# rajashree-srikanth/drone-sim-python

Hardware: AMD Instinct MI355X
Metric: trajectory-optimisations/sec (6-seg poly, 50 wpts) (higher is better)
Workload: dtype f64 residual/gradient + f32 MFMA J^T J

## Files before the change

### drone-sim-python_amd/csrc/fit_device.h

```cpp
#pragma once
#include <hip/hip_runtime.h>

#include "../../include/d2d.h"

#define FIT_G 9.81
#define FIT_OBS_K 2.0
#define FIT_OBS_ARGMAX 3.4538776394910684

typedef float f32x4 __attribute__((ext_vector_type(4)));
typedef float f32x2 __attribute__((ext_vector_type(2)));

__device__ __forceinline__ void wave_lds_sync() {
  __builtin_amdgcn_fence(__ATOMIC_RELEASE, "wavefront");
  __builtin_amdgcn_wave_barrier();
  __builtin_amdgcn_fence(__ATOMIC_ACQUIRE, "wavefront");
}

__device__ __forceinline__ double uniform_d(double v) {
  const int lo = __builtin_amdgcn_readfirstlane(__double2loint(v));
  const int hi = __builtin_amdgcn_readfirstlane(__double2hiint(v));
  return __hiloint2double(hi, lo);
}
__device__ __forceinline__ int uniform_i(int v) { return __builtin_amdgcn_readfirstlane(v); }

// ... 170 lines not shown
}

__device__ __forceinline__ ScenP load_scenp(const double *__restrict__ p) {
  ScenP s;
  s.cv = p[PR_CV]; s.cphi = p[PR_CPHI]; s.cobs = p[PR_COBS]; s.k0 = p[PR_K0]; s.k1 = p[PR_K1];
  s.cv2 = p[PR_CV2]; s.cphi2 = p[PR_CPHI2]; s.wb2 = p[PR_WB2]; s.wwp = p[PR_WWP]; s.wbnd = p[PR_WBND];
  s.vsp = p[PR_VSP]; s.wx = p[PR_WX]; s.wy = p[PR_WY]; s.phimax = p[PR_PHIMAX]; s.vmin = p[PR_VMIN]; s.vmax = p[PR_VMAX];
  s.o0x = p[PR_O0X]; s.o0y = p[PR_O0Y]; s.o1x = p[PR_O1X]; s.o1y = p[PR_O1Y];
  s.ccol = p[PR_CCOL]; s.kc = p[PR_KC]; s.pmask = (int)p[PR_PMASK];
  s.c0 = p[PR_C0]; s.c1 = p[PR_C1]; s.cphimax = p[PR_CPHIMAX];
  s.ext = p + PR_EXT;
  return s;
}

#define FIT_PK 8
__device__ __forceinline__ void prepk_entry(const double *__restrict__ pr, const double *__restrict__ Gp64, int K, int k,
                                            double o[FIT_PK]) {
#pragma unroll
  for (int d = 0; d < 3; ++d) {
    const double *gp = Gp64 + ((size_t)d * K + k) * 4;
    double ax = 0.0, ay = 0.0;
#pragma unroll
    for (int c = 0; c < 4; ++c) { ax = fma(gp[c], pr[PR_DX + c], ax); ay = fma(gp[c], pr[PR_DY + c], ay); }
    o[2 * d] = ax; o[2 * d + 1] = ay;
  }
  const int n1 = K / 2, n2 = K - n1;
  if (k < n1) {
    o[6] = (k == n1 - 1 && n1 > 1) ? pr[PR_P2X] : k * pr[PR_SAX] + pr[PR_X0];
    o[7] = (k == n1 - 1 && n1 > 1) ? pr[PR_P2Y] : k * pr[PR_SAY] + pr[PR_Y0];
  } else {
    const int i = k - n1;
    o[6] = (i == n2 - 1 && n2 > 1) ? pr[PR_X1] : i * pr[PR_SBX] + pr[PR_P2X];
    o[7] = (i == n2 - 1 && n2 > 1) ? pr[PR_Y1] : i * pr[PR_SBY] + pr[PR_P2Y];
  }
}

__device__ __forceinline__ int q_slot(int lane, int nq) { return lane < nq ? 2 * lane : 2 * (lane - nq) + 1; }

template <int NQ>
__device__ __forceinline__ void flat_outputs_pk(const FitGeom &g, const double *__restrict__ G64,
                                                const double *__restrict__ q, const double pk[FIT_PK], int k, double Y[6]) {
  typedef double __attribute__((ext_vector_type(2), may_alias)) f64x2a;
  const int nq = NQ ? NQ : g.nq, gstr = NQ ? NQ + 1 : g.gstr;
#pragma unroll
  for (int c = 0; c < 6; ++c) Y[c] = pk[c];
  const double *g0 = G64 + (size_t)k * gstr;
  const double *g1 = g0 + (size_t)g.K * gstr;
  const double *g2 = g1 + (size_t)g.K * gstr;
  int j = 0;
// ... 263 lines not shown
```

### drone-sim-python_amd/csrc/fit_kernels.hip

```cpp
#include <algorithm>
#include <chrono>
#include <cmath>
#include <cstdlib>
#include <cstring>
#include <vector>

#include "fit_device.h"
#include "fit_phases.h"
#include "fit_seg.h"
#include "fit_plan.h"
#include "fit_handout_prior.h"

#define FIT_EVAL_WPB_MAX 16
#define FIT_WPB_MAX 12
#define FIT_THREADS (64 * FIT_WPB_MAX)
#define FIT_LDS_BYTES (160 * 1024)
#define FIT_LDS_STATIC 256


struct FitLds {
  int G64, G32, wave0, wave_stride;
  int q, u, coef, cfd;
  int total;
};
// ... 23 lines not shown
}

static bool pick_eval_layout(int K, int nq, bool *g32_lds, int *wpb, int nds = 0) {
  for (int pass = 0; pass < 2; ++pass) {
    const bool in_lds = pass == 0;
    for (int w = FIT_EVAL_WPB_MAX; w >= (in_lds ? 4 : 1); --w)
      if (eval_lds_layout(K, nq, in_lds, w, nds).total <= FIT_LDS_BYTES - FIT_LDS_STATIC) { *g32_lds = in_lds; *wpb = w; return true; }
  }
  return false;
}

__device__ __forceinline__ void stage(void *dst, const void *src, int bytes) {
  double *d = reinterpret_cast<double *>(dst);
  const double *s = reinterpret_cast<const double *>(src);
  for (int i = threadIdx.x; i < bytes / 8; i += blockDim.x) d[i] = s[i];
}

__global__ void __launch_bounds__(256)
fit_prep_kernel(int B, int K, double duration, const double *__restrict__ scen, double *__restrict__ prep) {
  const int b = blockIdx.x * blockDim.x + threadIdx.x;
  if (b >= B) return;
  prep_row(scen + (size_t)b * D2D_SCEN_STRIDE, duration, K, prep + (size_t)b * FIT_PREP_STRIDE);
}

__global__ void __launch_bounds__(256)
fit_prepk_kernel(int B, int K, const double *__restrict__ prep, const double *__restrict__ Gp64, double *__restrict__ pk) {
  const long i = blockIdx.x * (long)blockDim.x + threadIdx.x;
  if (i >= (long)B * K) return;
  const int b = i / K, k = i - (long)b * K;
  double o[FIT_PK];
  prepk_entry(prep + (size_t)b * FIT_PREP_STRIDE, Gp64, K, k, o);
#pragma unroll
  for (int c = 0; c < FIT_PK; ++c) pk[((size_t)b * FIT_PK + c) * K + k] = o[c];
}

template <int NB, int NQ, bool G32_LDS>
__global__ void __launch_bounds__(64 * FIT_EVAL_WPB_MAX)
// ... 1434 lines not shown
#pragma unroll
      for (int t = 0; t < NT; ++t) acc[t] = f32x4{0.f, 0.f, 0.f, 0.f};
#pragma unroll
      for (int s = 0; s < D2D_FIT_MAX_S; ++s)
        if (s < sa.m.S) segment_project<NB, NQ>(nq, Zl32, s, bs[s][0], lane, acc);
      float *Hb = H_out + (size_t)b * NT * 256;
#pragma unroll
      for (int t = 0; t < NT; ++t)
#pragma unroll
        for (int r = 0; r < 4; ++r) Hb[(t * 4 + r) * 64 + lane] = acc[t][r];
    }
    wave_lds_sync();
  }
}

__global__ void __launch_bounds__(256)
fit_state_init_kernel(int B, int off, int stride, double *__restrict__ lm, int32_t *__restrict__ flags,
                      int32_t *__restrict__ queue) {
  const int i = blockIdx.x * blockDim.x + threadIdx.x;
  if (i == 0 && queue) { queue[0] = 0; queue[1] = 0; queue[2] = 0; queue[3] = 0; queue[4] = 0; queue[5] = 0; }
  if (i >= B) return;
  const int b = off + i * stride;
  lm[LM_STRIDE * b + 0] = D2D_LM_LAMBDA0; lm[LM_STRIDE * b + 1] = 2.0; lm[LM_STRIDE * b + 2] = 0.0; lm[LM_STRIDE * b + 3] = 0.0;
  lm[LM_STRIDE * b + 4] = 0.0; lm[LM_STRIDE * b + 5] = -1.0; lm[LM_STRIDE * b + 6] = 2.0; lm[LM_STRIDE * b + 7] = 0.0;
  flags[4 * b + FL_STATUS] = D2D_ST_RUNNING; flags[4 * b + FL_ITERS] = 0; flags[4 * b + FL_NEED] = 1;
  if (stride == 1) flags[4 * b + FL_NEVAL] = 0;
}


#define ORDER_BINS 2048
__global__ void __launch_bounds__(1024)
fit_order_kernel(int B, const int32_t *__restrict__ iters, int32_t *__restrict__ order) {
  __shared__ int hist[ORDER_BINS];
  for (int i = threadIdx.x; i < ORDER_BINS; i += blockDim.x) hist[i] = 0;
  __syncthreads();
  for (int b = threadIdx.x; b < B; b += blockDim.x) {
    int k = iters[b];
    k = k < 0 ? 0 : (k >= ORDER_BINS ? ORDER_BINS - 1 : k);
    atomicAdd(&hist[ORDER_BINS - 1 - k], 1);
  }
  __syncthreads();
// ... 9 lines not shown
      part[cur ^ 1][t] = v;
      cur ^= 1;
      __syncthreads();
    }
    const int excl = part[cur][t] - (h0 + h1);
    hist[2 * t] = excl; hist[2 * t + 1] = excl + h0;
  }
  __syncthreads();
  for (int b = threadIdx.x; b < B; b += blockDim.x) {
    int k = iters[b];
    k = k < 0 ? 0 : (k >= ORDER_BINS ? ORDER_BINS - 1 : k);
    order[atomicAdd(&hist[ORDER_BINS - 1 - k], 1)] = b;
  }
}

__global__ void __launch_bounds__(256)
fit_handout_key_kernel(int B, double duration, const double *__restrict__ scen, const float *__restrict__ tab, int32_t *__restrict__ key) {
  const int b = blockIdx.x * blockDim.x + threadIdx.x;
  if (b >= B) return;
  const double *r = scen + (size_t)b * D2D_SCEN_STRIDE;
  const double dx = r[D2D_SC_X1] - r[D2D_SC_X0], dy = r[D2D_SC_Y1] - r[D2D_SC_Y0];
  const double d = sqrt(dx * dx + dy * dy), D = r[D2D_SC_VREF] * duration;
  const double h = 0.5 * sqrt(fmax(D * D - d * d, 0.0));
  const double gl = r[D2D_SC_GOLEFT] > 0.0 ? 1.0 : (r[D2D_SC_GOLEFT] < 0.0 ? -1.0 : 0.0);
  const double beta = atan2(dy, dx), a = atan2(gl * h, 0.5 * d);
  const double TWO_PI = 6.283185307179586, PI = 3.141592653589793;
  auto wrap = [&](double v) { v = fmod(v + PI, TWO_PI); if (v < 0.0) v += TWO_PI; return v; };
  auto abin = [&](double v) { int i = (int)(wrap(v) * (D2D_HANDOUT_NB / TWO_PI)); return i < 0 ? 0 : (i >= D2D_HANDOUT_NB ? D2D_HANDOUT_NB - 1 : i); };
  const int b0 = abin(r[D2D_SC_PSI0] - (beta + a)), b1 = abin(r[D2D_SC_PSI1] - (beta - a));
  const double x = D > 0.0 ? d / D : 0.0;
  int bx = (int)floor((x - D2D_HANDOUT_X_LO) * (D2D_HANDOUT_ND / (D2D_HANDOUT_X_HI - D2D_HANDOUT_X_LO)));
  bx = bx < 0 ? 0 : (bx >= D2D_HANDOUT_ND ? D2D_HANDOUT_ND - 1 : bx);
  float k = tab[b0 * D2D_HANDOUT_ND + bx] + tab[(D2D_HANDOUT_NB + b1) * D2D_HANDOUT_ND + bx];
  if (!(k == k)) k = 0.f;
  int ki = (int)(8.f * (k + 40.f));
  key[b] = ki < 0 ? 0 : (ki >= ORDER_BINS ? ORDER_BINS - 1 : ki);
}

__global__ void __launch_bounds__(256)
fit_pos_kernel(int B, FitGeom g, const double *__restrict__ G64, const double *__restrict__ Gp64,
               const double *__restrict__ prep, const double *__restrict__ q, double *__restrict__ pos) {
  const long i = blockIdx.x * (long)blockDim.x + threadIdx.x;
  if (i >= (long)B * g.K) return;
  const int b = i / g.K, k = i - (long)b * g.K;
  const double *pr = prep + (size_t)b * FIT_PREP_STRIDE;
  const double *qa = q + (size_t)b * 2 * g.nq;
  const double *gp = Gp64 + (size_t)k * 4, *g0 = G64 + (size_t)k * g.gstr;
  double x = 0.0, y = 0.0;
  for (int c = 0; c < 4; ++c) { x = fma(gp[c], pr[PR_DX + c], x); y = fma(gp[c], pr[PR_DY + c], y); }
  for (int j = 0; j < g.nq; ++j) { x = fma(g0[j], qa[j], x); y = fma(g0[j], qa[g.nq + j], y); }
  pos[((size_t)b * 2) * g.K + k] = x;
// ... 40 lines not shown
    const int st = flags[4 * b + FL_STATUS];
    nr = (st == D2D_ST_CONVERGED || st == D2D_ST_STALLED) ? 0.0 : 1.0;
    ne = 0.5 * flags[4 * b + FL_NEVAL];
  }
  c = wave_sum(c); gm = wave_max(gm); nr = wave_sum(nr); ne = wave_sum(ne);
  if ((threadIdx.x & 63) == 0) {
    atomicAdd(&stats[0], c);
    atomicAdd(&stats[2], nr);
    atomicAdd(&stats[3], ne);
    atomicMax(reinterpret_cast<unsigned long long *>(&stats[1]), (unsigned long long)__double_as_longlong(gm));
  }
}

__global__ void __launch_bounds__(256)
fit_export_kernel(int B, const int32_t *__restrict__ flags, int32_t *__restrict__ iters,
                  int32_t *__restrict__ status) {
  const int b = blockIdx.x * blockDim.x + threadIdx.x;
  if (b >= B) return;
  if (iters) iters[b] = flags[4 * b + FL_ITERS];
  if (status) status[b] = flags[4 * b + FL_STATUS];
}

__global__ void __launch_bounds__(256)
fit_init_kernel(int B, int K, int nq, double duration, const double *__restrict__ Gp,
                const double *__restrict__ Pinit, const double *__restrict__ scen,
                double *__restrict__ q) {
  const int wave = threadIdx.x >> 6, lane = threadIdx.x & 63;
  const int b = blockIdx.x * 4 + wave;
  if (b >= B) return;
  const Scen s = load_scen(scen + (size_t)b * D2D_SCEN_STRIDE, duration);
  const int n = 2 * nq;
  for (int l = lane; l < n; l += 64) {
    const int ax = l >= nq, j = l - ax * nq;
// ... 120 lines not shown
  {
    int cap = 64;
    while (cap < B) cap <<= 1;
    SCRATCH_ALLOC(d_ring, (size_t)cap * sizeof(int32_t))
    pl->ring_cap = cap;
  }
  SCRATCH_ALLOC(d_cost, (size_t)B * sizeof(double))
  SCRATCH_ALLOC(d_lm, (size_t)B * LM_STRIDE * sizeof(double))
  SCRATCH_ALLOC(d_flags, (size_t)B * 4 * sizeof(int32_t))
#undef SCRATCH_ALLOC
  if (int rc = fit_knot_ensure(pl, B)) { free_scratch(pl); return rc; }
  pl->cap_B = B;
  return D2D_OK;
}

static int launch_prep(d2d_ctx *ctx, const d2d_fit_plan *pl, int B, const double *scen) {
  const_cast<d2d_fit_plan *>(pl)->rows_B = 0;
  hipLaunchKernelGGL(fit_prep_kernel, dim3((B + 63) / 64), dim3(64), 0, ctx->stream, B, pl->K, pl->duration, scen, pl->d_prep);
  hipLaunchKernelGGL(fit_prepk_kernel, dim3(((long)B * pl->K + 255) / 256), dim3(256), 0, ctx->stream, B, pl->K, pl->d_prep, pl->d_Gp, pl->d_pk);
  D2D_LAUNCH_CHECK();
  return D2D_OK;
}

static GroupArgs no_groups() { return GroupArgs{nullptr, 0, 0, 1, 0}; }

static int launch_eval(d2d_ctx *ctx, const d2d_fit_plan *pl, int B, const double *q,
                       int32_t *flags, double *cost, double *g, float *H, GroupArgs ga = no_groups(),
                       f32x4 *rows = nullptr) {
  const FitGeom gm = geom_of(pl);
  const FitLds L = eval_lds_layout(pl->K, pl->nq, pl->g32_lds, pl->wpb_eval, pl->nds);
  const int NB = (2 * pl->nq + 15) / 16;
  int nblk = (B + pl->wpb_eval - 1) / pl->wpb_eval;
  if (nblk > pl->n_cu) nblk = pl->n_cu;
  const dim3 grid(nblk), block(64 * pl->wpb_eval);
  static const int dbg = getenv("D2D_FIT_ABLATE") ? atoi(getenv("D2D_FIT_ABLATE")) : 0;
#define LAUNCH_EVAL(NBV, INLDS)                                                                    \
// ... 35 lines not shown
}

static int lm_slice(const d2d_fit_opts &o) { return o.slice > 0 ? o.slice : 0; }

static int solve_kernel_of(const d2d_fit_plan *pl, const d2d_fit_opts &o) {
  if (!pl->use_lm) return 2;
  return (pl->kn.wpb > 0 && o.mode == D2D_LM_MODE_MINPACK && lm_slice(o) <= 0) ? 1 : 0;
}

static const int32_t *handout_order(const d2d_fit_plan *pl, int B) {
  if (pl->order_B == B) return pl->d_order;
  if (pl->last_order == pl->d_order_pred && pl->last_order_B == B) return pl->d_order_pred;
  return nullptr;
}

static int launch_handout(d2d_ctx *ctx, d2d_fit_plan *pl, int B, const double *scen) {
  hipLaunchKernelGGL(fit_handout_key_kernel, dim3((B + 255) / 256), dim3(256), 0, ctx->stream, B, pl->duration, scen, pl->d_hprior, pl->d_hkey);
  hipLaunchKernelGGL(fit_order_kernel, dim3(1), dim3(1024), 0, ctx->stream, B, pl->d_hkey, pl->d_order_pred);
  D2D_LAUNCH_CHECK();
  return D2D_OK;
}

static int launch_lm(d2d_ctx *ctx, const d2d_fit_plan *pl, int B, double *q, const d2d_fit_opts &o, int iter_cap) {
  const FitGeom gm = geom_of(pl);
  const FusedLds L = fused_lds_layout(pl->K, pl->nq, 48, pl->wpb_lm);
  static const bool want_stamps = getenv("D2D_LM_STAMPS") != nullptr;
  static const bool want_times = getenv("D2D_LM_TIMES") != nullptr;
  std::chrono::steady_clock::time_point t0;
  if (want_times) { D2D_CHECK_HIP(hipStreamSynchronize(ctx->stream)); t0 = std::chrono::steady_clock::now(); }
  unsigned long long *stamps = want_stamps ? reinterpret_cast<unsigned long long *>(ctx->stats_dev + 8) : nullptr;
  if (want_stamps) D2D_CHECK_HIP(hipMemsetAsync(stamps, 0, 13 * sizeof(unsigned long long), ctx->stream));
  const int blocks = B < pl->n_cu ? B : pl->n_cu;
// ... 440 lines not shown
    out[2 * pl->prof_kind[i]] += ms;
    out[2 * pl->prof_kind[i] + 1] += 1.0;
  }
  return D2D_OK;
}


int d2d_fit_begin(d2d_ctx *ctx, d2d_fit_plan *pl, int B) {
  D2D_REQUIRE(ctx && pl, "d2d_fit_begin: null argument");
  D2D_REQUIRE(B >= 1, "d2d_fit_begin: B must be >= 1");
  if (pl->active_B != 0 && B > pl->cap_B) {
    d2d_set_error("d2d_fit_begin: a begin/iterate sequence of %d trajectories is in progress on this plan (finish it first)", pl->active_B);
    return D2D_ESTATE;
  }
  if (int rc = ensure_scratch(pl, B)) return rc;
  hipLaunchKernelGGL(fit_state_init_kernel, dim3((B + 255) / 256), dim3(256), 0, ctx->stream, B, 0, 1, pl->d_lm, pl->d_flags, ctx->counter_dev + 8);
  D2D_LAUNCH_CHECK();
  D2D_CHECK_HIP(hipMemsetAsync(pl->d_ring, 0xff, (size_t)pl->ring_cap * sizeof(int32_t), ctx->stream));
  pl->it_done = 0;
  pl->active_B = B;
  pl->solve_q = nullptr; pl->solve_kernel = -1;
  pl->last_order = nullptr; pl->last_order_B = 0;
  pl->prep_valid_for = nullptr;
  pl->rows_B = 0;
  pl->last_slice = 0; pl->last_running = -1;
  pl->gsweeps_R = 0;
  return D2D_OK;
}

int d2d_fit_iterate(d2d_ctx *ctx, d2d_fit_plan *pl, int B, const double *scen, double *q,
                    const d2d_fit_opts *opts, int n_iters, int32_t *n_running) {
  D2D_REQUIRE(ctx && pl && scen && q, "d2d_fit_iterate: null argument");
  if (pl->active_B != B) { d2d_set_error("d2d_fit_iterate: call d2d_fit_begin(B=%d) first", B); return D2D_ESTATE; }
  const d2d_fit_opts o = opts_or_default(opts);
  D2D_REQUIRE(o.max_iter >= 1 && n_iters >= 1, "d2d_fit_iterate: max_iter and n_iters must be >= 1");
  const dim3 g1((B + 255) / 256), b1(256);
  if (pl->prep_valid_for != scen) {
    if (int rc = launch_prep(ctx, pl, B, scen)) return rc;
    pl->prep_valid_for = scen;
  }
  if ((pl->use_lm || pl->use_long) && pl->n_group <= 1) {
    const int sk = solve_kernel_of(pl, o);
    if (pl->solve_kernel < 0) {
      pl->solve_q = q; pl->solve_kernel = sk;
      pl->last_order = pl->order_B == B ? pl->d_order : nullptr;
      if (pl->order_B != B && pl->has_prior && o.handout == D2D_HANDOUT_PREDICTED && o.mode == D2D_LM_MODE_MINPACK && B > 8 * pl->n_cu) {
        if (int rc = launch_handout(ctx, pl, B, scen)) return rc;
        pl->last_order = pl->d_order_pred;
      }
      pl->last_order_B = pl->last_order ? B : 0;
    } else {
      if (q != pl->solve_q) {
        d2d_set_error("d2d_fit_iterate: q differs from the buffer this solve started on (between d2d_fit_begin and d2d_fit_finish the solve owns q)");
        return D2D_EINVAL;
      }
      if (sk != pl->solve_kernel) {
        d2d_set_error("d2d_fit_iterate: these options (mode / slice) would move the solve in progress to another kernel; finish it and begin again");
        return D2D_ESTATE;
      }
    }
    int budget = o.max_iter - pl->it_done;
    if (budget > n_iters) budget = n_iters;
// ... 49 lines not shown
      return D2D_ESTATE;
    }
    if (int rc = launch_lm(ctx, pl, B, q, pl->last_opts, cap)) return rc;
  }
}

int d2d_fit_finish(d2d_ctx *ctx, d2d_fit_plan *pl, int B, const double *scen, const double *q,
                   double *cost, int32_t *iters, int32_t *status, double *stats) {
  D2D_REQUIRE(ctx && pl && scen && q, "d2d_fit_finish: null argument");
  if (pl->active_B != B) { d2d_set_error("d2d_fit_finish: call d2d_fit_begin(B=%d) first", B); return D2D_ESTATE; }
  if (pl->solve_q != nullptr && q != pl->solve_q) {
    d2d_set_error("d2d_fit_finish: q differs from the buffer the d2d_fit_iterate calls of this solve worked on");
    return D2D_EINVAL;
  }
  const dim3 g1((B + 255) / 256), b1(256);
  if (pl->prep_valid_for != scen) {
    if (int rc = launch_prep(ctx, pl, B, scen)) return rc;
    pl->prep_valid_for = scen;
  }
  if (pl->use_lm && pl->n_group <= 1 && pl->last_slice > 0 && pl->it_done > 0)
    if (int rc = sweep_up_sliced(ctx, pl, B, const_cast<double *>(q))) return rc;
  if (!((pl->use_lm || pl->use_long) && pl->n_group <= 1 && pl->it_done > 0))
    if (int rc = launch_eval(ctx, pl, B, q, nullptr, pl->d_cost, pl->d_g, nullptr)) return rc;
  if (cost) D2D_CHECK_HIP(hipMemcpyAsync(cost, pl->d_cost, (size_t)B * sizeof(double), hipMemcpyDeviceToDevice, ctx->stream));
  hipLaunchKernelGGL(fit_export_kernel, g1, b1, 0, ctx->stream, B, pl->d_flags, iters, status);
  D2D_LAUNCH_CHECK();
  if (stats) {
    D2D_CHECK_HIP(hipMemsetAsync(ctx->stats_dev, 0, 4 * sizeof(double), ctx->stream));
    hipLaunchKernelGGL(fit_stats_kernel, dim3((B + 63) / 64), dim3(64), 0, ctx->stream, B, 2 * pl->nq, pl->d_cost, pl->d_g, pl->d_flags, ctx->stats_dev);
    D2D_LAUNCH_CHECK();
    D2D_CHECK_HIP(hipMemcpyAsync(ctx->stats_host, ctx->stats_dev, 4 * sizeof(double), hipMemcpyDeviceToHost, ctx->stream));
  }
  D2D_CHECK_HIP(hipStreamSynchronize(ctx->stream));
  if (stats)
    for (int i = 0; i < 4; ++i) stats[i] = ctx->stats_host[i];
  pl->active_B = 0;
  return D2D_OK;
}

int d2d_fit_solve(d2d_ctx *ctx, const d2d_fit_plan *plc, int B, const double *scen, double *q,
                  const d2d_fit_opts *opts, double *cost, int32_t *iters, int32_t *status, double *stats) {
  D2D_REQUIRE(ctx && plc && scen && q, "d2d_fit_solve: null argument");
// ... 250 lines not shown
```

### drone-sim-python_amd/csrc/fit_knot.hip

```cpp
#include <cstdlib>
#include <vector>

#include "fit_phases.h"
#include "fit_plan.h"

#define KN_WPB_MAX 8
#define KN_LDS_BYTES (160 * 1024)
#define KN_N 48
#define KN_NE 56
#define KN_WV_KNOT 10
#define KN_US 10
#define KN_GTOL_SCALE 0.1
#define KN_SEG_MAX 11
#define KN_IMG_LS (KN_N + 4)

namespace {

#define LAUNDER_S(v) do { (v) = __builtin_amdgcn_readfirstlane(v); asm volatile("" : "+s"(v)); } while (0)

struct KnotGeom {
  int K, S, smax;
  int k0[D2D_FIT_MAX_S + 2];
};

// ... 284 lines not shown
  __device__ __forceinline__ f32x4 damp(int j0) const {
#ifdef KN_ABL_DAMP
    return f32x4{lam, lam, lam, lam};
#endif
    const float *mdrow = reinterpret_cast<const float *>(lds + row_off);
    return lam != 0.f ? lds_get<f32x4>(mdrow + j0) : f32x4{0.f, 0.f, 0.f, 0.f};
  }
};

}
template <> struct nd_is_banded<KnotMetric> { static constexpr bool value = true; };
namespace {

template <bool STAMPS, bool SEG9>
__global__ void __launch_bounds__(64 * KN_WPB_MAX)
fit_lm_knot_kernel(int B, KnotGeom kg, KnotLds L, d2d_fit_opts opts, int iter_cap, KnotDev T, const double *__restrict__ pk,
                   const double *__restrict__ prep, double *q_io, double *cost_io, double *g_io, double *lm, int32_t *flags,
                   int32_t *queue, const int32_t *__restrict__ order, int prio_at, double *u_io, unsigned long long *__restrict__ stamps,
                   float *dbg) {
  unsigned long long st_acc[8] = {0, 0, 0, 0, 0, 0, 0, 0}, st_last = 0;
#define KN_STAMP(i)                                                     \
  if (STAMPS) {                                                         \
    const unsigned long long t_ = __builtin_amdgcn_s_memtime();         \
    st_acc[i] += t_ - st_last;                                          \
    st_last = t_;                                                       \
  }
  extern __shared__ __attribute__((aligned(16))) unsigned char lds[];
  constexpr int N = KN_N;
  stage(lds + L.Hb64, T.Hb64, kg.K * KN_HB_STRIDE * 8);
  stage(lds + L.Hb32, T.Hb32, kg.K * 32 * 4);
  stage(lds + L.Wseg, T.Wseg, D2D_FIT_MAX_S * 4 * 64 * 4);
  stage(lds + L.Md32, T.Md32, N * N * 4);
// ... 30 lines not shown
  };
  auto seg_of_lane = [&]() -> int {
    int lj = lane;
    LAUNDER(lj);
    int sg = 0;
#pragma unroll
    for (int s = 1; s < D2D_FIT_MAX_S; ++s) sg += (lj >= kg.k0[s] && s < kg.S) ? 1 : 0;
    return sg;
  };
  auto msc_of_lane = [&]() -> double {
    int l = lane;
    LAUNDER(l);
    return reinterpret_cast<const double *>(lds + L.Msc)[l < N ? kn_entry_of(l) : 0];
  };
  for (int i = lane; i < 9 * 8; i += 64) sfull[i] = 0.f;
  KnotMetric metric;
  metric.lds = lds; metric.sfull_off = L.wave0 + wave * L.wave_stride + L.sfull; metric.md32_off = L.Md32; metric.mr32_off = L.Mr32;
  metric.lane = lane; metric.lam = 0.f; metric.scale = 0.f; metric.row_off = 0;

  const int stride = gridDim.x * (blockDim.x >> 6);
  auto take = [&](bool first) -> int {
    if (first) {
      const int bi = blockIdx.x + gridDim.x * wave;
      if (bi >= B) return -1;
      return order ? __builtin_amdgcn_readfirstlane(order[bi]) : bi;
    }
    int t = -1;
    int32_t *qp = queue;
    asm volatile("" : "+s"(qp));
    if (lane == 0 && stride + __hip_atomic_load(qp, __ATOMIC_RELAXED, __HIP_MEMORY_SCOPE_AGENT) < B) {
// ... 5 lines not shown
  if (STAMPS) st_last = __builtin_amdgcn_s_memtime();
  bool first_take = true;
  for (;;) {
    int b = take(first_take);
    first_take = false;
    if (b < 0) break;
    if (flags[4 * b + FL_STATUS] != D2D_ST_RUNNING) continue;
    const double *prow = prep + (size_t)b * FIT_PREP_STRIDE;
    double *lmb = lm + (size_t)b * LM_STRIDE;
    int iters = uniform_i(flags[4 * b + FL_ITERS]);
    {
      int lane_ld = lane;
      LAUNDER(lane_ld);
      for (int i = lane_ld; i < FIT_PREP_STRIDE; i += 64) sp[i] = prow[i];
      double wpx = 0.0, wpy = 0.0;
      if (lane_ld < kg.K) { wpx = pk[((size_t)b * FIT_PK + 6) * kg.K + lane_ld]; wpy = pk[((size_t)b * FIT_PK + 7) * kg.K + lane_ld]; }
      park[lane_ld] = wpx; park[64 + lane_ld] = wpy;
    }
    wave_lds_sync();
    double ui = 0.0;
    auto u0_of_lane = [&]() -> double { int l = lane; LAUNDER(l); return park[128 + l]; };
    {
      double u0i = 0.0;
      int lane_ld = lane;
      LAUNDER(lane_ld);
      const int e_ld = kn_entry_all(lane_ld);
      if (lane_ld < KN_NE) {
        const double *pu = T.Pu + (size_t)e_ld * 4;
        const double *ed = sp + (((e_ld >> 2) & 1) ? PR_DY : PR_DX);
        u0i = fma(pu[0], ed[0], fma(pu[1], ed[1], fma(pu[2], ed[2], pu[3] * ed[3])));
      }
// ... 341 lines not shown
        g_io[(size_t)b * N + lane_io] = gq;
        if (status == D2D_ST_RUNNING) u_io[(size_t)b * 64 + lane_io] = ui;
      }
      const double gmax = uniform_d(wave_max(fabs(gq)));
      if (lane == 0) {
        int bs = b;
        LAUNDER_S(bs);
        double *lmb = lm + (size_t)bs * LM_STRIDE;
        int *flags_b = flags + 4 * (size_t)bs;
        cost_io[bs] = c;
        lmb[2] = gmax; lmb[3] = so_rows ? 1.0 : 0.0;
        if (phase == 0) { lmb[4] = V_mp_par; lmb[5] = V_mp_delta; } else { lmb[0] = V_lam; lmb[1] = V_nu; }
        lmb[6] = (double)(phase | (mp.first << 1) | ((mp.calm & 0x3fff) << 2) | (mp.slow << 16));
        lmb[7] = lmb[7] + (double)mp.nfac;
        flags_b[FL_STATUS] = status; flags_b[FL_ITERS] = iters; flags_b[FL_NEED] = 1;
        flags_b[FL_NEVAL] = flags_b[FL_NEVAL] + nev;
      }
    }
    __builtin_amdgcn_s_setprio(0);
    KN_STAMP(0)
  }
  if (queue != nullptr && lane == 0) {
    if (atomicAdd(queue + 1, 1) == stride - 1) { queue[0] = 0; queue[1] = 0; queue[2] = 0; queue[3] = 0; queue[4] = 0; }
  }
  if (STAMPS && lane == 0)
    for (int i = 0; i < 8; ++i) atomicAdd(&stamps[i], st_acc[i]);
#undef KN_STAMP
#undef V_lam
#undef V_nu
#undef V_mp_par
#undef V_mp_delta
// ... 56 lines not shown

void fit_knot_plan_free(d2d_fit_plan *pl) {
  auto &kn = pl->kn;
  void *p[] = {kn.d_Hb64, kn.d_Hb32, kn.d_Wseg, kn.d_Md32, kn.d_Mrow32, kn.d_Mi32, kn.d_Bq, kn.d_BiT, kn.d_Binv, kn.d_Minv, kn.d_Pu, kn.d_msc, kn.d_u};
  for (void *q : p)
    if (q) hipFree(q);
  kn.d_Hb64 = kn.d_Bq = kn.d_BiT = kn.d_Binv = kn.d_Minv = kn.d_Pu = kn.d_msc = kn.d_u = nullptr;
  kn.d_Hb32 = kn.d_Wseg = kn.d_Md32 = kn.d_Mrow32 = kn.d_Mi32 = nullptr;
  kn.wpb = 0;
}

int fit_knot_ensure(d2d_fit_plan *pl, int cap_B) {
  auto &kn = pl->kn;
  if (kn.wpb == 0) return D2D_OK;
  if (kn.d_u) { hipFree(kn.d_u); kn.d_u = nullptr; }
  D2D_CHECK_HIP(hipMalloc(&kn.d_u, (size_t)cap_B * 64 * sizeof(double)));
  D2D_CHECK_HIP(hipMemset(kn.d_u, 0, (size_t)cap_B * 64 * sizeof(double)));
  return D2D_OK;
}

int fit_knot_launch(d2d_ctx *ctx, d2d_fit_plan *pl, int B, double *q, const d2d_fit_opts &o, int iter_cap, const int32_t *order, int prio_at) {
  auto &kn = pl->kn;
  KnotGeom kg;
  kg.K = pl->K; kg.S = pl->S; kg.smax = 0;
  for (int s = 0; s <= D2D_FIT_MAX_S + 1; ++s) kg.k0[s] = kn.k0[s < D2D_FIT_MAX_S + 2 ? s : D2D_FIT_MAX_S + 1];
  for (int j = 0; j < pl->S; ++j)
    if (kn.k0[j + 1] - kn.k0[j] > kg.smax) kg.smax = kn.k0[j + 1] - kn.k0[j];
  const KnotLds L = knot_lds_layout(pl->K, kn.wpb);
  KnotDev T{kn.d_Hb64, kn.d_Bq, kn.d_BiT, kn.d_Binv, kn.d_Minv, kn.d_Pu, kn.d_msc, kn.d_Hb32, kn.d_Wseg, kn.d_Md32, kn.d_Mrow32, kn.d_Mi32};
  static const bool want_stamps = getenv("D2D_LM_STAMPS") != nullptr || getenv("D2D_KNOT_DEBUG") != nullptr;
  unsigned long long *stamps = want_stamps ? reinterpret_cast<unsigned long long *>(ctx->stats_dev + 8) : nullptr;
  if (want_stamps) D2D_CHECK_HIP(hipMemsetAsync(stamps, 0, 8 * sizeof(unsigned long long), ctx->stream));
  const int blocks = B < pl->n_cu ? B : pl->n_cu;
  int32_t *queue = ctx->counter_dev + 8;
  float *dbg = nullptr;
  if (getenv("D2D_KNOT_DEBUG")) D2D_CHECK_HIP(hipMalloc(&dbg, (size_t)B * (KN_N * KN_N + 4 * KN_N) * sizeof(float)));
#define KN_LAUNCH(ST, S9)                                                                                                                  \
  hipLaunchKernelGGL((fit_lm_knot_kernel<ST, S9>), dim3(blocks), dim3(64 * kn.wpb), L.total, ctx->stream, B, kg, L, o, iter_cap, T, pl->d_pk, \
                     pl->d_prep, q, pl->d_cost, pl->d_g, pl->d_lm, pl->d_flags, queue, order, prio_at, kn.d_u, stamps, dbg)
  const bool seg9 = kg.smax <= 9;
  if (want_stamps) { if (seg9) KN_LAUNCH(true, true); else KN_LAUNCH(true, false); }
  else { if (seg9) KN_LAUNCH(false, true); else KN_LAUNCH(false, false); }
#undef KN_LAUNCH
  D2D_LAUNCH_CHECK();
  if (dbg) {
    std::vector<float> h((size_t)B * (KN_N * KN_N + 4 * KN_N));
    D2D_CHECK_HIP(hipMemcpyAsync(h.data(), dbg, h.size() * sizeof(float), hipMemcpyDeviceToHost, ctx->stream));
    D2D_CHECK_HIP(hipStreamSynchronize(ctx->stream));
    if (FILE *f = fopen(getenv("D2D_KNOT_DEBUG"), "wb")) { fwrite(h.data(), sizeof(float), h.size(), f); fclose(f); }
    hipFree(dbg);
  }
  if (want_stamps) {
    unsigned long long h[8];
    D2D_CHECK_HIP(hipMemcpyAsync(h, stamps, sizeof(h), hipMemcpyDeviceToHost, ctx->stream));
    D2D_CHECK_HIP(hipStreamSynchronize(ctx->stream));
// ... 10 lines not shown
```

### drone-sim-python_amd/csrc/fit_plan.h

```cpp
#pragma once
#include <vector>

#include "common.h"

enum { FL_STATUS = 0, FL_ITERS = 1, FL_NEED = 2, FL_NEVAL = 3 };
#define LM_STRIDE 8

#define KN_HB_STRIDE 34
struct KnotTables {
  int NE = 0, NV = 0;
  int k0[D2D_FIT_MAX_S + 2] = {0};
  std::vector<double> Hb64, Bq, BiT, Binv, Minv, Mrow, Pu, msc;
  std::vector<float> Hb32, Wseg, Md32, Mrow32, Mi32;
  double *d_Hb64 = nullptr, *d_Bq = nullptr, *d_BiT = nullptr, *d_Binv = nullptr, *d_Minv = nullptr, *d_Pu = nullptr, *d_msc = nullptr;
  float *d_Hb32 = nullptr, *d_Wseg = nullptr, *d_Md32 = nullptr, *d_Mrow32 = nullptr, *d_Mi32 = nullptr;
  double *d_u = nullptr;
  int wpb = 0;
};

struct d2d_fit_plan {
  int device;
  int S, K, nq;
  double duration, T;
  double wref[3];
  std::vector<double> G, Gp, Z, Zp, Pinit, G0tG0;
  std::vector<double> Lw, Pe;
  KnotTables kn;
  std::vector<int> seg;
  std::vector<double> tau;
  std::vector<double> Zl, Zlp, sx;
  int seg_S = 0, seg_nchunk = 0, seg_l0[7] = {0}, seg_k0[6] = {0}, seg_Ks[6] = {0};
  double *d_G = nullptr;
  double *d_GT = nullptr;
// ... 20 lines not shown
  float *d_rows = nullptr;
  int rows_B = 0;
  int32_t *d_order = nullptr;
  int order_B = 0;
  float *d_hprior = nullptr;
  bool has_prior = false;
  int32_t *d_hkey = nullptr;
  int32_t *d_order_pred = nullptr;
  const int32_t *last_order = nullptr;
  int last_order_B = 0;
  int32_t *d_ring = nullptr;
  int ring_cap = 0;
  int gorder_R = 0, gsweeps_R = 0;
  int n_group = 1, nds = 0;
  const double *prep_valid_for = nullptr;
  bool g32_lds = true;
  int wpb_eval = 8, wpb_step = 8, wpb_lm = 0;
  bool use_lm = false;
  bool use_long = false;
  bool split_ok = true;
  int n_cu = 256;
  int kernel_req = D2D_FIT_KERNEL_AUTO, long_tables = -1;
  int it_done = 0, active_B = 0;
  const double *solve_q = nullptr;
  int solve_kernel = -1;
  int last_slice = 0, last_running = -1;
  d2d_fit_opts last_opts = {};
  bool prof_on = false;
  std::vector<hipEvent_t> prof_ev;
  std::vector<int> prof_kind;
// ... 10 lines not shown
```

Baseline: 1.640 million.

## Fuse prologue kernels, defer state init, and fold stats into export

Merges the prep, state-init and handout-key kernels into one prologue kernel, and defers state init to the first iterate or export call. The knot solver now computes waypoints inline instead of reading the pk table, so the prepk launch can be skipped on that path. Per-wave cost, gradient and count partials are accumulated during the solve and reduced by an extra block of the export kernel, which also copies cost. This replaces the separate memcpy, memset and stats kernel and drops the ring memset. The aim is fewer kernel launches and less small-op overhead per batch, in exchange for more flag-driven bookkeeping that could go stale.

```diff
diff --git a/drone-sim-python_amd/csrc/fit_device.h b/drone-sim-python_amd/csrc/fit_device.h
--- a/drone-sim-python_amd/csrc/fit_device.h
+++ b/drone-sim-python_amd/csrc/fit_device.h
@@ -208,6 +208,18 @@
 }
 
 #define FIT_PK 8
+__device__ __forceinline__ void prepk_waypoint(const double *pr, int K, int k, double &wx, double &wy) {
+  const int n1 = K / 2, n2 = K - n1;
+  if (k < n1) {
+    wx = (k == n1 - 1 && n1 > 1) ? pr[PR_P2X] : k * pr[PR_SAX] + pr[PR_X0];
+    wy = (k == n1 - 1 && n1 > 1) ? pr[PR_P2Y] : k * pr[PR_SAY] + pr[PR_Y0];
+  } else {
+    const int i = k - n1;
+    wx = (i == n2 - 1 && n2 > 1) ? pr[PR_X1] : i * pr[PR_SBX] + pr[PR_P2X];
+    wy = (i == n2 - 1 && n2 > 1) ? pr[PR_Y1] : i * pr[PR_SBY] + pr[PR_P2Y];
+  }
+}
+
 __device__ __forceinline__ void prepk_entry(const double *__restrict__ pr, const double *__restrict__ Gp64, int K, int k,
                                             double o[FIT_PK]) {
 #pragma unroll
@@ -218,15 +230,7 @@
     for (int c = 0; c < 4; ++c) { ax = fma(gp[c], pr[PR_DX + c], ax); ay = fma(gp[c], pr[PR_DY + c], ay); }
     o[2 * d] = ax; o[2 * d + 1] = ay;
   }
-  const int n1 = K / 2, n2 = K - n1;
-  if (k < n1) {
-    o[6] = (k == n1 - 1 && n1 > 1) ? pr[PR_P2X] : k * pr[PR_SAX] + pr[PR_X0];
-    o[7] = (k == n1 - 1 && n1 > 1) ? pr[PR_P2Y] : k * pr[PR_SAY] + pr[PR_Y0];
-  } else {
-    const int i = k - n1;
-    o[6] = (i == n2 - 1 && n2 > 1) ? pr[PR_X1] : i * pr[PR_SBX] + pr[PR_P2X];
-    o[7] = (i == n2 - 1 && n2 > 1) ? pr[PR_Y1] : i * pr[PR_SBY] + pr[PR_P2Y];
-  }
+  prepk_waypoint(pr, K, k, o[6], o[7]);
 }
 
 __device__ __forceinline__ int q_slot(int lane, int nq) { return lane < nq ? 2 * lane : 2 * (lane - nq) + 1; }
diff --git a/drone-sim-python_amd/csrc/fit_kernels.hip b/drone-sim-python_amd/csrc/fit_kernels.hip
--- a/drone-sim-python_amd/csrc/fit_kernels.hip
+++ b/drone-sim-python_amd/csrc/fit_kernels.hip
@@ -61,13 +61,6 @@
   double *d = reinterpret_cast<double *>(dst);
   const double *s = reinterpret_cast<const double *>(src);
   for (int i = threadIdx.x; i < bytes / 8; i += blockDim.x) d[i] = s[i];
-}
-
-__global__ void __launch_bounds__(256)
-fit_prep_kernel(int B, int K, double duration, const double *__restrict__ scen, double *__restrict__ prep) {
-  const int b = blockIdx.x * blockDim.x + threadIdx.x;
-  if (b >= B) return;
-  prep_row(scen + (size_t)b * D2D_SCEN_STRIDE, duration, K, prep + (size_t)b * FIT_PREP_STRIDE);
 }
 
 __global__ void __launch_bounds__(256)
@@ -1532,17 +1525,21 @@
   }
 }
 
+__device__ __forceinline__ void state_init_fit(int b, bool reset_neval, double *__restrict__ lm, int32_t *__restrict__ flags) {
+  lm[LM_STRIDE * b + 0] = D2D_LM_LAMBDA0; lm[LM_STRIDE * b + 1] = 2.0; lm[LM_STRIDE * b + 2] = 0.0; lm[LM_STRIDE * b + 3] = 0.0;
+  lm[LM_STRIDE * b + 4] = 0.0; lm[LM_STRIDE * b + 5] = -1.0; lm[LM_STRIDE * b + 6] = 2.0; lm[LM_STRIDE * b + 7] = 0.0;
+  flags[4 * b + FL_STATUS] = D2D_ST_RUNNING; flags[4 * b + FL_ITERS] = 0; flags[4 * b + FL_NEED] = 1;
+  if (reset_neval) flags[4 * b + FL_NEVAL] = 0;
+}
+__device__ __forceinline__ void queue_init(int32_t *queue) { queue[0] = 0; queue[1] = 0; queue[2] = 0; queue[3] = 0; queue[4] = 0; queue[5] = 0; }
+
 __global__ void __launch_bounds__(256)
 fit_state_init_kernel(int B, int off, int stride, double *__restrict__ lm, int32_t *__restrict__ flags,
                       int32_t *__restrict__ queue) {
   const int i = blockIdx.x * blockDim.x + threadIdx.x;
-  if (i == 0 && queue) { queue[0] = 0; queue[1] = 0; queue[2] = 0; queue[3] = 0; queue[4] = 0; queue[5] = 0; }
+  if (i == 0 && queue) queue_init(queue);
   if (i >= B) return;
-  const int b = off + i * stride;
-  lm[LM_STRIDE * b + 0] = D2D_LM_LAMBDA0; lm[LM_STRIDE * b + 1] = 2.0; lm[LM_STRIDE * b + 2] = 0.0; lm[LM_STRIDE * b + 3] = 0.0;
-  lm[LM_STRIDE * b + 4] = 0.0; lm[LM_STRIDE * b + 5] = -1.0; lm[LM_STRIDE * b + 6] = 2.0; lm[LM_STRIDE * b + 7] = 0.0;
-  flags[4 * b + FL_STATUS] = D2D_ST_RUNNING; flags[4 * b + FL_ITERS] = 0; flags[4 * b + FL_NEED] = 1;
-  if (stride == 1) flags[4 * b + FL_NEVAL] = 0;
+  state_init_fit(off + i * stride, stride == 1, lm, flags);
 }
 
 
@@ -1582,11 +1579,7 @@
   }
 }
 
-__global__ void __launch_bounds__(256)
-fit_handout_key_kernel(int B, double duration, const double *__restrict__ scen, const float *__restrict__ tab, int32_t *__restrict__ key) {
-  const int b = blockIdx.x * blockDim.x + threadIdx.x;
-  if (b >= B) return;
-  const double *r = scen + (size_t)b * D2D_SCEN_STRIDE;
+__device__ __forceinline__ int handout_key(const double *__restrict__ r, double duration, const float *__restrict__ tab) {
   const double dx = r[D2D_SC_X1] - r[D2D_SC_X0], dy = r[D2D_SC_Y1] - r[D2D_SC_Y0];
   const double d = sqrt(dx * dx + dy * dy), D = r[D2D_SC_VREF] * duration;
   const double h = 0.5 * sqrt(fmax(D * D - d * d, 0.0));
@@ -1601,8 +1594,19 @@
   bx = bx < 0 ? 0 : (bx >= D2D_HANDOUT_ND ? D2D_HANDOUT_ND - 1 : bx);
   float k = tab[b0 * D2D_HANDOUT_ND + bx] + tab[(D2D_HANDOUT_NB + b1) * D2D_HANDOUT_ND + bx];
   if (!(k == k)) k = 0.f;
-  int ki = (int)(8.f * (k + 40.f));
-  key[b] = ki < 0 ? 0 : (ki >= ORDER_BINS ? ORDER_BINS - 1 : ki);
+  const int ki = (int)(8.f * (k + 40.f));
+  return ki < 0 ? 0 : (ki >= ORDER_BINS ? ORDER_BINS - 1 : ki);
+}
+
+__global__ void __launch_bounds__(64)
+fit_prologue_kernel(int B, int K, double duration, const double *__restrict__ scen, double *__restrict__ prep, double *__restrict__ lm,
+                    int32_t *__restrict__ flags, int32_t *__restrict__ queue, const float *__restrict__ tab, int32_t *__restrict__ key) {
+  const int b = blockIdx.x * blockDim.x + threadIdx.x;
+  if (b == 0 && lm && queue) queue_init(queue);
+  if (b >= B) return;
+  if (lm) state_init_fit(b, true, lm, flags);
+  if (key) key[b] = handout_key(scen + (size_t)b * D2D_SCEN_STRIDE, duration, tab);
+  if (prep) prep_row(scen + (size_t)b * D2D_SCEN_STRIDE, duration, K, prep + (size_t)b * FIT_PREP_STRIDE);
 }
 
 __global__ void __launch_bounds__(256)
@@ -1673,9 +1677,27 @@
 
 __global__ void __launch_bounds__(256)
 fit_export_kernel(int B, const int32_t *__restrict__ flags, int32_t *__restrict__ iters,
-                  int32_t *__restrict__ status) {
+                  int32_t *__restrict__ status, const double *__restrict__ cost_in = nullptr, double *__restrict__ cost = nullptr,
+                  const double *__restrict__ part = nullptr, int n_part = 0, double *__restrict__ stats = nullptr) {
+  if (part != nullptr && blockIdx.x == gridDim.x - 1) {
+    __shared__ double red[4][256];
+    double c = 0.0, g = 0.0, nr = 0.0, ne = 0.0;
+    for (int w = threadIdx.x; w < n_part; w += 256) { c += part[4 * w]; g = fmax(g, part[4 * w + 1]); nr += part[4 * w + 2]; ne += part[4 * w + 3]; }
+    red[0][threadIdx.x] = c; red[1][threadIdx.x] = g; red[2][threadIdx.x] = nr; red[3][threadIdx.x] = ne;
+    __syncthreads();
+    for (int d = 128; d > 0; d >>= 1) {
+      if ((int)threadIdx.x < d) {
+        red[0][threadIdx.x] += red[0][threadIdx.x + d]; red[1][threadIdx.x] = fmax(red[1][threadIdx.x], red[1][threadIdx.x + d]);
+        red[2][threadIdx.x] += red[2][threadIdx.x + d]; red[3][threadIdx.x] += red[3][threadIdx.x + d];
+      }
+      __syncthreads();
+    }
+    if (threadIdx.x == 0) { stats[0] = red[0][0]; stats[1] = red[1][0]; stats[2] = red[2][0]; stats[3] = 0.5 * red[3][0]; }
+    return;
+  }
   const int b = blockIdx.x * blockDim.x + threadIdx.x;
   if (b >= B) return;
+  if (cost) cost[b] = cost_in[b];
   if (iters) iters[b] = flags[4 * b + FL_ITERS];
   if (status) status[b] = flags[4 * b + FL_STATUS];
 }
@@ -1826,12 +1848,25 @@
   return D2D_OK;
 }
 
+static int launch_prologue(d2d_ctx *ctx, d2d_fit_plan *pl, int B, const double *scen, bool want_prep, bool want_pk, bool want_key, bool allow_init = true) {
+  const bool init = allow_init && pl->state_pending;
+  if (want_prep) { pl->rows_B = 0; pl->pk_valid = false; }
+  if (init || want_prep || want_key) {
+    hipLaunchKernelGGL(fit_prologue_kernel, dim3((B + 63) / 64), dim3(64), 0, ctx->stream, B, pl->K, pl->duration, scen,
+                       want_prep ? pl->d_prep : nullptr, init ? pl->d_lm : nullptr, pl->d_flags, ctx->counter_dev + 8,
+                       pl->d_hprior, want_key ? pl->d_hkey : nullptr);
+    if (init) pl->state_pending = false;
+  }
+  if (want_pk) {
+    hipLaunchKernelGGL(fit_prepk_kernel, dim3(((long)B * pl->K + 255) / 256), dim3(256), 0, ctx->stream, B, pl->K, pl->d_prep, pl->d_Gp, pl->d_pk);
+    pl->pk_valid = true;
+  }
+  D2D_LAUNCH_CHECK();
+  return D2D_OK;
+}
+
 static int launch_prep(d2d_ctx *ctx, const d2d_fit_plan *pl, int B, const double *scen) {
-  const_cast<d2d_fit_plan *>(pl)->rows_B = 0;
-  hipLaunchKernelGGL(fit_prep_kernel, dim3((B + 63) / 64), dim3(64), 0, ctx->stream, B, pl->K, pl->duration, scen, pl->d_prep);
-  hipLaunchKernelGGL(fit_prepk_kernel, dim3(((long)B * pl->K + 255) / 256), dim3(256), 0, ctx->stream, B, pl->K, pl->d_prep, pl->d_Gp, pl->d_pk);
-  D2D_LAUNCH_CHECK();
-  return D2D_OK;
+  return launch_prologue(ctx, const_cast<d2d_fit_plan *>(pl), B, scen, true, true, false, false);
 }
 
 static GroupArgs no_groups() { return GroupArgs{nullptr, 0, 0, 1, 0}; }
@@ -1897,8 +1932,7 @@
   return nullptr;
 }
 
-static int launch_handout(d2d_ctx *ctx, d2d_fit_plan *pl, int B, const double *scen) {
-  hipLaunchKernelGGL(fit_handout_key_kernel, dim3((B + 255) / 256), dim3(256), 0, ctx->stream, B, pl->duration, scen, pl->d_hprior, pl->d_hkey);
+static int launch_handout(d2d_ctx *ctx, d2d_fit_plan *pl, int B) {
   hipLaunchKernelGGL(fit_order_kernel, dim3(1), dim3(1024), 0, ctx->stream, B, pl->d_hkey, pl->d_order_pred);
   D2D_LAUNCH_CHECK();
   return D2D_OK;
@@ -2369,9 +2403,8 @@
     return D2D_ESTATE;
   }
   if (int rc = ensure_scratch(pl, B)) return rc;
-  hipLaunchKernelGGL(fit_state_init_kernel, dim3((B + 255) / 256), dim3(256), 0, ctx->stream, B, 0, 1, pl->d_lm, pl->d_flags, ctx->counter_dev + 8);
-  D2D_LAUNCH_CHECK();
-  D2D_CHECK_HIP(hipMemsetAsync(pl->d_ring, 0xff, (size_t)pl->ring_cap * sizeof(int32_t), ctx->stream));
+  pl->state_pending = true;
+  pl->kn.stats_ready = false;
   pl->it_done = 0;
   pl->active_B = B;
   pl->solve_q = nullptr; pl->solve_kernel = -1;
@@ -2390,17 +2423,23 @@
   const d2d_fit_opts o = opts_or_default(opts);
   D2D_REQUIRE(o.max_iter >= 1 && n_iters >= 1, "d2d_fit_iterate: max_iter and n_iters must be >= 1");
   const dim3 g1((B + 255) / 256), b1(256);
-  if (pl->prep_valid_for != scen) {
-    if (int rc = launch_prep(ctx, pl, B, scen)) return rc;
+  const bool persistent = (pl->use_lm || pl->use_long) && pl->n_group <= 1;
+  const bool want_key = persistent && pl->solve_kernel < 0 && pl->order_B != B && pl->has_prior && o.handout == D2D_HANDOUT_PREDICTED &&
+                        o.mode == D2D_LM_MODE_MINPACK && B > 8 * pl->n_cu;
+  {
+    const bool want_prep = pl->prep_valid_for != scen;
+    const bool want_pk = !(persistent && solve_kernel_of(pl, o) == 1) && (want_prep || !pl->pk_valid);
+    if (pl->state_pending || want_prep || want_pk || want_key)
+      if (int rc = launch_prologue(ctx, pl, B, scen, want_prep, want_pk, want_key)) return rc;
     pl->prep_valid_for = scen;
   }
-  if ((pl->use_lm || pl->use_long) && pl->n_group <= 1) {
+  if (persistent) {
     const int sk = solve_kernel_of(pl, o);
     if (pl->solve_kernel < 0) {
       pl->solve_q = q; pl->solve_kernel = sk;
       pl->last_order = pl->order_B == B ? pl->d_order : nullptr;
-      if (pl->order_B != B && pl->has_prior && o.handout == D2D_HANDOUT_PREDICTED && o.mode == D2D_LM_MODE_MINPACK && B > 8 * pl->n_cu) {
-        if (int rc = launch_handout(ctx, pl, B, scen)) return rc;
+      if (want_key) {
+        if (int rc = launch_handout(ctx, pl, B)) return rc;
         pl->last_order = pl->d_order_pred;
       }
       pl->last_order_B = pl->last_order ? B : 0;
@@ -2480,18 +2519,31 @@
     return D2D_EINVAL;
   }
   const dim3 g1((B + 255) / 256), b1(256);
-  if (pl->prep_valid_for != scen) {
-    if (int rc = launch_prep(ctx, pl, B, scen)) return rc;
+  const bool solved = (pl->use_lm || pl->use_long) && pl->n_group <= 1 && pl->it_done > 0;
+  {
+    const bool want_prep = pl->prep_valid_for != scen;
+    const bool want_pk = (!solved || pl->solve_kernel != 1) && (want_prep || !pl->pk_valid);
+    if (pl->state_pending || want_prep || want_pk)
+      if (int rc = launch_prologue(ctx, pl, B, scen, want_prep, want_pk, false)) return rc;
     pl->prep_valid_for = scen;
   }
   if (pl->use_lm && pl->n_group <= 1 && pl->last_slice > 0 && pl->it_done > 0)
     if (int rc = sweep_up_sliced(ctx, pl, B, const_cast<double *>(q))) return rc;
-  if (!((pl->use_lm || pl->use_long) && pl->n_group <= 1 && pl->it_done > 0))
+  if (!solved)
     if (int rc = launch_eval(ctx, pl, B, q, nullptr, pl->d_cost, pl->d_g, nullptr)) return rc;
-  if (cost) D2D_CHECK_HIP(hipMemcpyAsync(cost, pl->d_cost, (size_t)B * sizeof(double), hipMemcpyDeviceToDevice, ctx->stream));
-  hipLaunchKernelGGL(fit_export_kernel, g1, b1, 0, ctx->stream, B, pl->d_flags, iters, status);
-  D2D_LAUNCH_CHECK();
-  if (stats) {
+  const bool one_launch = solved && pl->solve_kernel == 1 && pl->kn.stats_ready;
+  if (one_launch) {
+    const int n_part = (B < pl->n_cu ? B : pl->n_cu) * pl->kn.wpb;
+    hipLaunchKernelGGL(fit_export_kernel, dim3(g1.x + (stats ? 1 : 0)), b1, 0, ctx->stream, B, pl->d_flags, iters, status, pl->d_cost, cost,
+                       stats ? knot_stat_slots(pl->kn, B) : nullptr, n_part, ctx->stats_dev);
+    D2D_LAUNCH_CHECK();
+    if (stats) D2D_CHECK_HIP(hipMemcpyAsync(ctx->stats_host, ctx->stats_dev, 4 * sizeof(double), hipMemcpyDeviceToHost, ctx->stream));
+  } else {
+    if (cost) D2D_CHECK_HIP(hipMemcpyAsync(cost, pl->d_cost, (size_t)B * sizeof(double), hipMemcpyDeviceToDevice, ctx->stream));
+    hipLaunchKernelGGL(fit_export_kernel, g1, b1, 0, ctx->stream, B, pl->d_flags, iters, status);
+    D2D_LAUNCH_CHECK();
+  }
+  if (stats && !one_launch) {
     D2D_CHECK_HIP(hipMemsetAsync(ctx->stats_dev, 0, 4 * sizeof(double), ctx->stream));
     hipLaunchKernelGGL(fit_stats_kernel, dim3((B + 63) / 64), dim3(64), 0, ctx->stream, B, 2 * pl->nq, pl->d_cost, pl->d_g, pl->d_flags, ctx->stats_dev);
     D2D_LAUNCH_CHECK();
diff --git a/drone-sim-python_amd/csrc/fit_knot.hip b/drone-sim-python_amd/csrc/fit_knot.hip
--- a/drone-sim-python_amd/csrc/fit_knot.hip
+++ b/drone-sim-python_amd/csrc/fit_knot.hip
@@ -4,7 +4,6 @@
 #include "fit_phases.h"
 #include "fit_plan.h"
 
-#define KN_WPB_MAX 8
 #define KN_LDS_BYTES (160 * 1024)
 #define KN_N 48
 #define KN_NE 56
@@ -322,8 +321,7 @@
 
 template <bool STAMPS, bool SEG9>
 __global__ void __launch_bounds__(64 * KN_WPB_MAX)
-fit_lm_knot_kernel(int B, KnotGeom kg, KnotLds L, d2d_fit_opts opts, int iter_cap, KnotDev T, const double *__restrict__ pk,
-                   const double *__restrict__ prep, double *q_io, double *cost_io, double *g_io, double *lm, int32_t *flags,
+fit_lm_knot_kernel(int B, KnotGeom kg, KnotLds L, d2d_fit_opts opts, int iter_cap, KnotDev T, const double *__restrict__ prep, double *q_io, double *cost_io, double *g_io, double *lm, int32_t *flags,
                    int32_t *queue, const int32_t *__restrict__ order, int prio_at, double *u_io, unsigned long long *__restrict__ stamps,
                    float *dbg) {
   unsigned long long st_acc[8] = {0, 0, 0, 0, 0, 0, 0, 0}, st_last = 0;
@@ -384,6 +382,7 @@
     return reinterpret_cast<const double *>(lds + L.Msc)[l < N ? kn_entry_of(l) : 0];
   };
   for (int i = lane; i < 9 * 8; i += 64) sfull[i] = 0.f;
+  if (SEG9 && lane < 4) u_io[(size_t)B * 64 + 4 * (size_t)(blockIdx.x * (blockDim.x >> 6) + wave) + lane] = 0.0;
   KnotMetric metric;
   metric.lds = lds; metric.sfull_off = L.wave0 + wave * L.wave_stride + L.sfull; metric.md32_off = L.Md32; metric.mr32_off = L.Mr32;
   metric.lane = lane; metric.lam = 0.f; metric.scale = 0.f; metric.row_off = 0;
@@ -419,7 +418,7 @@
       LAUNDER(lane_ld);
       for (int i = lane_ld; i < FIT_PREP_STRIDE; i += 64) sp[i] = prow[i];
       double wpx = 0.0, wpy = 0.0;
-      if (lane_ld < kg.K) { wpx = pk[((size_t)b * FIT_PK + 6) * kg.K + lane_ld]; wpy = pk[((size_t)b * FIT_PK + 7) * kg.K + lane_ld]; }
+      if (lane_ld < kg.K) prepk_waypoint(prow, kg.K, lane_ld, wpx, wpy);
       park[lane_ld] = wpx; park[64 + lane_ld] = wpy;
     }
     wave_lds_sync();
@@ -791,7 +790,13 @@
         lmb[6] = (double)(phase | (mp.first << 1) | ((mp.calm & 0x3fff) << 2) | (mp.slow << 16));
         lmb[7] = lmb[7] + (double)mp.nfac;
         flags_b[FL_STATUS] = status; flags_b[FL_ITERS] = iters; flags_b[FL_NEED] = 1;
-        flags_b[FL_NEVAL] = flags_b[FL_NEVAL] + nev;
+        const int nev_all = flags_b[FL_NEVAL] + nev;
+        flags_b[FL_NEVAL] = nev_all;
+        if (SEG9) {
+          double *slot = u_io + (size_t)B * 64 + 4 * (size_t)(blockIdx.x * (blockDim.x >> 6) + (threadIdx.x >> 6));
+          slot[0] += c; slot[1] = fmax(slot[1], gmax);
+          slot[2] += (status == D2D_ST_CONVERGED || status == D2D_ST_STALLED) ? 0.0 : 1.0; slot[3] += (double)nev_all;
+        }
       }
     }
     __builtin_amdgcn_s_setprio(0);
@@ -878,8 +883,9 @@
   auto &kn = pl->kn;
   if (kn.wpb == 0) return D2D_OK;
   if (kn.d_u) { hipFree(kn.d_u); kn.d_u = nullptr; }
-  D2D_CHECK_HIP(hipMalloc(&kn.d_u, (size_t)cap_B * 64 * sizeof(double)));
-  D2D_CHECK_HIP(hipMemset(kn.d_u, 0, (size_t)cap_B * 64 * sizeof(double)));
+  const size_t n_u = (size_t)cap_B * 64 + (size_t)pl->n_cu * KN_WPB_MAX * 4;
+  D2D_CHECK_HIP(hipMalloc(&kn.d_u, n_u * sizeof(double)));
+  D2D_CHECK_HIP(hipMemset(kn.d_u, 0, n_u * sizeof(double)));
   return D2D_OK;
 }
 
@@ -900,9 +906,10 @@
   float *dbg = nullptr;
   if (getenv("D2D_KNOT_DEBUG")) D2D_CHECK_HIP(hipMalloc(&dbg, (size_t)B * (KN_N * KN_N + 4 * KN_N) * sizeof(float)));
 #define KN_LAUNCH(ST, S9)                                                                                                                  \
-  hipLaunchKernelGGL((fit_lm_knot_kernel<ST, S9>), dim3(blocks), dim3(64 * kn.wpb), L.total, ctx->stream, B, kg, L, o, iter_cap, T, pl->d_pk, \
+  hipLaunchKernelGGL((fit_lm_knot_kernel<ST, S9>), dim3(blocks), dim3(64 * kn.wpb), L.total, ctx->stream, B, kg, L, o, iter_cap, T, \
                      pl->d_prep, q, pl->d_cost, pl->d_g, pl->d_lm, pl->d_flags, queue, order, prio_at, kn.d_u, stamps, dbg)
   const bool seg9 = kg.smax <= 9;
+  kn.stats_ready = seg9 && pl->it_done == 0 && iter_cap >= o.max_iter;
   if (want_stamps) { if (seg9) KN_LAUNCH(true, true); else KN_LAUNCH(true, false); }
   else { if (seg9) KN_LAUNCH(false, true); else KN_LAUNCH(false, false); }
 #undef KN_LAUNCH
diff --git a/drone-sim-python_amd/csrc/fit_plan.h b/drone-sim-python_amd/csrc/fit_plan.h
--- a/drone-sim-python_amd/csrc/fit_plan.h
+++ b/drone-sim-python_amd/csrc/fit_plan.h
@@ -7,6 +7,7 @@
 #define LM_STRIDE 8
 
 #define KN_HB_STRIDE 34
+#define KN_WPB_MAX 8
 struct KnotTables {
   int NE = 0, NV = 0;
   int k0[D2D_FIT_MAX_S + 2] = {0};
@@ -16,7 +17,10 @@
   float *d_Hb32 = nullptr, *d_Wseg = nullptr, *d_Md32 = nullptr, *d_Mrow32 = nullptr, *d_Mi32 = nullptr;
   double *d_u = nullptr;
   int wpb = 0;
+  bool stats_ready = false;
 };
+
+inline double *knot_stat_slots(const KnotTables &kn, int B) { return kn.d_u + (size_t)B * 64; }
 
 struct d2d_fit_plan {
   int device;
@@ -67,6 +71,8 @@
   int gorder_R = 0, gsweeps_R = 0;
   int n_group = 1, nds = 0;
   const double *prep_valid_for = nullptr;
+  bool pk_valid = false;
+  bool state_pending = false;
   bool g32_lds = true;
   int wpb_eval = 8, wpb_step = 8, wpb_lm = 0;
   bool use_lm = false;
```

Result: faster. 1.670 million, median of 6 (+1.8%).
